# anuragranj/cc

Measured on NVIDIA H100. Metric: train-step triplets/sec at 256x832x6lvl, higher is better.
Workload: dtype f32

## Files before the change

cc_b200/csrc/conv_tc.cu:

```cuda
#include "conv.cuh"

#ifndef CCB_CPU_SIM

#include <cuda.h>
#include <cudaTypedefs.h>

namespace ccb {

constexpr int TC_M = 128;
constexpr int TC_NMAX = 128;
constexpr int TC_KC = 8;
constexpr int TC_MAX_STAGES = 4;
constexpr int TC_PRODUCERS = 128;
constexpr int TC_CONSUMER_WARPS = 8;
constexpr int TC_THREADS = TC_PRODUCERS + 32 * TC_CONSUMER_WARPS;
constexpr int TC_MAX_TAPS = 49;
constexpr int TC_PRODUCER_REGS = 72, TC_CONSUMER_REGS = 216;

struct TcArgs {
    CUtensorMap wmap;
    const float* x;
    const float* bias;
    const float* res;
    float* out;
    int B, Cin, Hin, Win;
    int Ntot;
    int Hout, Wout;
    int Hc, Wc;
    int out_stride, out_oy, out_ox;
    int in_stride;
    int ntaps, cpad, Kp;
    int M;
    int act;
    float slope;
    int ktiles, kt_per_split, splits;
    float* partial;
    int tiles_m, tiles_n, units;
    long long out_numel;
    int depth, b_tile_bytes;
    signed char off_y[TC_MAX_TAPS], off_x[TC_MAX_TAPS];
};

__device__ __forceinline__ uint32_t smem_u32(const void* p) { return (uint32_t)__cvta_generic_to_shared(p); }

__device__ __forceinline__ void mbar_init(uint64_t* bar, uint32_t count) {
    asm volatile("mbarrier.init.shared::cta.b64 [%0], %1;" ::"r"(smem_u32(bar)), "r"(count));
}
__device__ __forceinline__ void mbar_arrive(uint64_t* bar) {
    asm volatile("mbarrier.arrive.shared::cta.b64 _, [%0];" ::"r"(smem_u32(bar)) : "memory");
}
__device__ __forceinline__ bool mbar_try(uint64_t* bar, uint32_t parity) {
    uint32_t ok;
    asm volatile(
        "{\n\t"
        ".reg .pred p;\n\t"
        "mbarrier.try_wait.parity.shared::cta.b64 p, [%1], %2;\n\t"
        "selp.u32 %0, 1, 0, p;\n\t"
        "}"
        : "=r"(ok)
        : "r"(smem_u32(bar)), "r"(parity)
        : "memory");
    return ok != 0;
}
__device__ __forceinline__ void mbar_wait(uint64_t* bar, uint32_t parity) {
    uint32_t spins = 0;
    while (!mbar_try(bar, parity)) {
        if (++spins > (1u << 26)) asm volatile("trap;");
    }
}
__device__ __forceinline__ void fence_proxy_async() { asm volatile("fence.proxy.async.shared::cta;" ::: "memory"); }
__device__ __forceinline__ void fence_barrier_init() { asm volatile("fence.mbarrier_init.release.cluster;" ::: "memory"); }
__device__ __forceinline__ void mbar_arrive_expect_tx(uint64_t* bar, uint32_t bytes) {
    asm volatile("mbarrier.arrive.expect_tx.shared::cta.b64 _, [%0], %1;" ::"r"(smem_u32(bar)), "r"(bytes) : "memory");
}
__device__ __forceinline__ void tma_load_3d(void* dst, const CUtensorMap* map, uint64_t* bar, int c0, int c1, int c2) {
    asm volatile(
        "cp.async.bulk.tensor.3d.shared::cluster.global.mbarrier::complete_tx::bytes [%0], [%1, {%3, %4, %5}], [%2];"
        ::"r"(smem_u32(dst)), "l"(map), "r"(smem_u32(bar)), "r"(c0), "r"(c1), "r"(c2)
        : "memory");
}
__device__ __forceinline__ void tma_prefetch_map(const CUtensorMap* map) {
    asm volatile("prefetch.tensormap [%0];" ::"l"(map) : "memory");
}
__device__ __forceinline__ void cp_async_4(uint32_t dst, const float* src, bool valid) {
    asm volatile("cp.async.ca.shared.global [%0], [%1], 4, %2;" ::"r"(dst), "l"(src), "r"(valid ? 4 : 0) : "memory");
}
__device__ __forceinline__ void cp_async_arrive(uint64_t* bar) {
    asm volatile("cp.async.mbarrier.arrive.noinc.shared::cta.b64 [%0];" ::"r"(smem_u32(bar)) : "memory");
}
__device__ __forceinline__ void cp_async_wait_all() { asm volatile("cp.async.wait_all;" ::: "memory"); }
__device__ __forceinline__ void cp_async_16(uint32_t dst, const void* src, bool valid) {
    asm volatile("cp.async.cg.shared.global [%0], [%1], 16, %2;" ::"r"(dst), "l"(src), "r"(valid ? 16 : 0) : "memory");
}
__device__ __forceinline__ float tf32_hi(float x) {
    uint32_t r;
    asm("cvt.rna.tf32.f32 %0, %1;" : "=r"(r) : "f"(x));
    return __uint_as_float(r);
}

__device__ __forceinline__ uint64_t wg_desc(uint32_t saddr) {
    return (uint64_t)((saddr & 0x3FFFF) >> 4) | ((uint64_t)1 << 16) | ((uint64_t)(1024 >> 4) << 32) | ((uint64_t)1 << 62);
}
__device__ __forceinline__ void wg_fence() { asm volatile("wgmma.fence.sync.aligned;" ::: "memory"); }
__device__ __forceinline__ void wg_commit() { asm volatile("wgmma.commit_group.sync.aligned;" ::: "memory"); }
template <int PENDING>
__device__ __forceinline__ void wg_wait() { asm volatile("wgmma.wait_group.sync.aligned %0;" ::"n"(PENDING) : "memory"); }
template <int R>
__device__ __forceinline__ void wg_fence_regs(float (&d)[R]) {
#pragma unroll
    for (int i = 0; i < R; ++i) asm volatile("" : "+f"(d[i])::"memory");
}
template <int K, int R>
__device__ __forceinline__ void wg_fence_regs(uint32_t (&d)[K][R]) {
#pragma unroll
    for (int k = 0; k < K; ++k)
#pragma unroll
        for (int i = 0; i < R; ++i) asm volatile("" : "+r"(d[k][i])::"memory");
}

__device__ __forceinline__ void wgmma_tf32_rs_n16(float (&d)[8], const uint32_t (&a)[4], uint64_t db) {
    asm volatile(
        "{\n\t.reg .pred p;\n\tsetp.ne.b32 p, 1, 0;\n\t"
        "wgmma.mma_async.sync.aligned.m64n16k8.f32.tf32.tf32 "
        "{%0, %1, %2, %3, %4, %5, %6, %7}, "
        "{%8, %9, %10, %11}, %12, p, 1, 1;\n\t}"
        : "+f"(d[0]), "+f"(d[1]), "+f"(d[2]), "+f"(d[3]), "+f"(d[4]), "+f"(d[5]), "+f"(d[6]), "+f"(d[7])
        : "r"(a[0]), "r"(a[1]), "r"(a[2]), "r"(a[3]), "l"(db));
}
__device__ __forceinline__ void wgmma_tf32_rs_n32(float (&d)[16], const uint32_t (&a)[4], uint64_t db) {
    asm volatile(
        "{\n\t.reg .pred p;\n\tsetp.ne.b32 p, 1, 0;\n\t"
        "wgmma.mma_async.sync.aligned.m64n32k8.f32.tf32.tf32 "
        "{%0, %1, %2, %3, %4, %5, %6, %7, %8, %9, %10, %11, %12, %13, %14, %15}, "
        "{%16, %17, %18, %19}, %20, p, 1, 1;\n\t}"
        : "+f"(d[0]), "+f"(d[1]), "+f"(d[2]), "+f"(d[3]), "+f"(d[4]), "+f"(d[5]), "+f"(d[6]), "+f"(d[7]),
          "+f"(d[8]), "+f"(d[9]), "+f"(d[10]), "+f"(d[11]), "+f"(d[12]), "+f"(d[13]), "+f"(d[14]), "+f"(d[15])
        : "r"(a[0]), "r"(a[1]), "r"(a[2]), "r"(a[3]), "l"(db));
}
__device__ __forceinline__ void wgmma_tf32_rs_n64(float (&d)[32], const uint32_t (&a)[4], uint64_t db) {
    asm volatile(
        "{\n\t.reg .pred p;\n\tsetp.ne.b32 p, 1, 0;\n\t"
        "wgmma.mma_async.sync.aligned.m64n64k8.f32.tf32.tf32 "
        "{%0, %1, %2, %3, %4, %5, %6, %7, %8, %9, %10, %11, %12, %13, %14, %15,"
        " %16, %17, %18, %19, %20, %21, %22, %23, %24, %25, %26, %27, %28, %29, %30, %31}, "
        "{%32, %33, %34, %35}, %36, p, 1, 1;\n\t}"
        : "+f"(d[0]), "+f"(d[1]), "+f"(d[2]), "+f"(d[3]), "+f"(d[4]), "+f"(d[5]), "+f"(d[6]), "+f"(d[7]),
          "+f"(d[8]), "+f"(d[9]), "+f"(d[10]), "+f"(d[11]), "+f"(d[12]), "+f"(d[13]), "+f"(d[14]), "+f"(d[15]),
          "+f"(d[16]), "+f"(d[17]), "+f"(d[18]), "+f"(d[19]), "+f"(d[20]), "+f"(d[21]), "+f"(d[22]), "+f"(d[23]),
          "+f"(d[24]), "+f"(d[25]), "+f"(d[26]), "+f"(d[27]), "+f"(d[28]), "+f"(d[29]), "+f"(d[30]), "+f"(d[31])
        : "r"(a[0]), "r"(a[1]), "r"(a[2]), "r"(a[3]), "l"(db));
}
__device__ __forceinline__ void wgmma_tf32_rs_n128(float (&d)[64], const uint32_t (&a)[4], uint64_t db) {
    asm volatile(
        "{\n\t.reg .pred p;\n\tsetp.ne.b32 p, 1, 0;\n\t"
        "wgmma.mma_async.sync.aligned.m64n128k8.f32.tf32.tf32 "
        "{%0, %1, %2, %3, %4, %5, %6, %7, %8, %9, %10, %11, %12, %13, %14, %15,"
        " %16, %17, %18, %19, %20, %21, %22, %23, %24, %25, %26, %27, %28, %29, %30, %31,"
        " %32, %33, %34, %35, %36, %37, %38, %39, %40, %41, %42, %43, %44, %45, %46, %47,"
        " %48, %49, %50, %51, %52, %53, %54, %55, %56, %57, %58, %59, %60, %61, %62, %63}, "
        "{%64, %65, %66, %67}, %68, p, 1, 1;\n\t}"
        : "+f"(d[0]), "+f"(d[1]), "+f"(d[2]), "+f"(d[3]), "+f"(d[4]), "+f"(d[5]), "+f"(d[6]), "+f"(d[7]),
          "+f"(d[8]), "+f"(d[9]), "+f"(d[10]), "+f"(d[11]), "+f"(d[12]), "+f"(d[13]), "+f"(d[14]), "+f"(d[15]),
          "+f"(d[16]), "+f"(d[17]), "+f"(d[18]), "+f"(d[19]), "+f"(d[20]), "+f"(d[21]), "+f"(d[22]), "+f"(d[23]),
          "+f"(d[24]), "+f"(d[25]), "+f"(d[26]), "+f"(d[27]), "+f"(d[28]), "+f"(d[29]), "+f"(d[30]), "+f"(d[31]),
          "+f"(d[32]), "+f"(d[33]), "+f"(d[34]), "+f"(d[35]), "+f"(d[36]), "+f"(d[37]), "+f"(d[38]), "+f"(d[39]),
          "+f"(d[40]), "+f"(d[41]), "+f"(d[42]), "+f"(d[43]), "+f"(d[44]), "+f"(d[45]), "+f"(d[46]), "+f"(d[47]),
          "+f"(d[48]), "+f"(d[49]), "+f"(d[50]), "+f"(d[51]), "+f"(d[52]), "+f"(d[53]), "+f"(d[54]), "+f"(d[55]),
          "+f"(d[56]), "+f"(d[57]), "+f"(d[58]), "+f"(d[59]), "+f"(d[60]), "+f"(d[61]), "+f"(d[62]), "+f"(d[63])
        : "r"(a[0]), "r"(a[1]), "r"(a[2]), "r"(a[3]), "l"(db));
}
template <int NT>
__device__ __forceinline__ void wgmma_tf32_rs(float (&d)[NT / 2], const uint32_t (&a)[4], uint64_t db) {
    if constexpr (NT == 16) wgmma_tf32_rs_n16(d, a, db);
    else if constexpr (NT == 32) wgmma_tf32_rs_n32(d, a, db);
    else if constexpr (NT == 64) wgmma_tf32_rs_n64(d, a, db);
    else wgmma_tf32_rs_n128(d, a, db);
}

template <int R> __device__ __forceinline__ void wg_regs_dec() { asm volatile("setmaxnreg.dec.sync.aligned.u32 %0;" ::"n"(R)); }
template <int R> __device__ __forceinline__ void wg_regs_inc() { asm volatile("setmaxnreg.inc.sync.aligned.u32 %0;" ::"n"(R)); }

constexpr int TC_TILE_BYTES = TC_KC * TC_M * 16;
constexpr int TC_SMEM_MAX = 227 * 1024;

__device__ __forceinline__ int tile_idx(int row, int chunk) { return row * TC_KC + (chunk ^ (row & 7)); }

__device__ __forceinline__ void tc_split_store(unsigned char* hi, unsigned char* lo, int idx, float4 x) {
    float4 h, l;
    h.x = tf32_hi(x.x); h.y = tf32_hi(x.y); h.z = tf32_hi(x.z); h.w = tf32_hi(x.w);
    ((float4*)hi)[idx] = h;
    l.x = tf32_hi(x.x - h.x); l.y = tf32_hi(x.y - h.y); l.z = tf32_hi(x.z - h.z); l.w = tf32_hi(x.w - h.w);
    ((float4*)lo)[idx] = l;
}

template <typename T> struct TcTiles { T a_hi, a_lo, b_hi, b_lo; };

struct TcRing {
    unsigned char* smem;
    int depth, stage_bytes, b_tile_bytes;
    uint64_t *full, *empty;

    template <typename T>
    __device__ __forceinline__ TcTiles<T> tiles(T base, int s) const {
        const T st = base + s * stage_bytes;
        return {st, st + TC_TILE_BYTES, st + 2 * TC_TILE_BYTES, st + 2 * TC_TILE_BYTES + b_tile_bytes};
    }
    __device__ __forceinline__ TcTiles<unsigned char*> acquire(int it, int s) const {
        if (it >= depth) mbar_wait(&empty[s], ((it / depth) - 1) & 1);
        return tiles(smem, s);
    }
    __device__ __forceinline__ void publish(int s) const { fence_proxy_async(); mbar_arrive(&full[s]); }
};

__device__ __forceinline__ TcRing tc_ring(int depth, int b_tile_bytes, int full_arrivals) {
    CCB_PDL_TRIGGER();
    extern __shared__ __align__(1024) unsigned char smem_raw[];
    unsigned char* smem = smem_raw + ((1024u - (smem_u32(smem_raw) & 1023u)) & 1023u);
    const int stage_bytes = 2 * TC_TILE_BYTES + 2 * b_tile_bytes;
    uint64_t* full = (uint64_t*)(smem + depth * stage_bytes);
    const TcRing r = {smem, depth, stage_bytes, b_tile_bytes, full, full + TC_MAX_STAGES};
    if (threadIdx.x == 0) {
        for (int s = 0; s < depth; ++s) { mbar_init(&r.full[s], full_arrivals); mbar_init(&r.empty[s], TC_CONSUMER_WARPS); }
        fence_barrier_init();
    }
    __syncthreads();
    CCB_PDL_SYNC();
    return r;
}

__device__ __forceinline__ int tc_acc_row(int wg, int wq, int lane, int half) { return wg * 64 + wq * 16 + (lane >> 2) + half * 8; }
__device__ __forceinline__ int tc_acc_col(int lane, int i, int e) { return 8 * i + 2 * (lane & 3) + e; }
__device__ __forceinline__ int tc_acc_reg(int i, int half, int e) { return 4 * i + 2 * half + e; }

struct TcAFrag { uint32_t hi[TC_KC / 2][4], lo[TC_KC / 2][4]; };

__device__ __forceinline__ int tc_a_idx(int r, int k) { return k * TC_M + (r ^ (8 * (k & 3))); }
struct TcAFprop {
    __device__ __forceinline__ static int off(int r0, int t) { return tc_a_idx(r0, t) * 4; }
    __device__ __forceinline__ static int at(int off, int h, int j) { return (off ^ (32 * h)) + 2048 * j; }
};
struct TcAWgrad {
    __device__ __forceinline__ static int idx(int r, int k) { return 32 * r + (k ^ (4 * (r & 7))); }
    __device__ __forceinline__ static int off(int r0, int t) { return idx(r0, t) * 4; }
    __device__ __forceinline__ static int at(int off, int h, int j) { return (off + 1024 * h) ^ (16 * j); }
};
template <typename L>
__device__ __forceinline__ void tc_load_a(const unsigned char* tile, int off, float (&v)[2][8]) {
#pragma unroll
    for (int h = 0; h < 2; ++h)
#pragma unroll
        for (int j = 0; j < 8; ++j) v[h][j] = *(const float*)(tile + L::at(off, h, j));
}
__device__ __forceinline__ void tc_split_a(const float (&v)[2][8], TcAFrag& f) {
#pragma unroll
    for (int ks = 0; ks < TC_KC / 2; ++ks)
#pragma unroll
        for (int i = 0; i < 4; ++i) {
            const float x = v[i & 1][2 * ks + (i >> 1)], h = tf32_hi(x);
            f.hi[ks][i] = __float_as_uint(h);
            f.lo[ks][i] = __float_as_uint(tf32_hi(x - h));
        }
}

__device__ __forceinline__ void tc_consumer_sync() { asm volatile("bar.sync 1, %0;" ::"n"(32 * TC_CONSUMER_WARPS) : "memory"); }

struct TcFpropFeed {
    static constexpr bool split_b = false;
    __device__ __forceinline__ void prep_b(const TcTiles<unsigned char*>&) const {}
};

template <int NT, typename L, typename Feed>
__device__ __forceinline__ void tc_consume_rs(const TcRing& ring, int g, int nkt, int wg, int wq, int lane, const Feed& feed,
                                              float (&acc)[NT / 2]) {
    constexpr bool split_ahead = NT < 128;
#pragma unroll
    for (int j = 0; j < NT / 2; ++j) acc[j] = 0.f;
    const uint32_t base = smem_u32(ring.smem);
    const int a_off = L::off(wg * 64 + wq * 16 + (lane >> 2), lane & 3);
    TcAFrag cur, nxt;
    auto take = [&](int st, uint32_t ph, TcAFrag& f) {
        mbar_wait(&ring.full[st], ph);
        const TcTiles<unsigned char*> t = ring.tiles(ring.smem, st);
        float v[2][8];
        tc_load_a<L>(t.a_hi, a_off, v);
        tc_split_a(v, f);
        if constexpr (Feed::split_b) {
            feed.prep_b(t);
            fence_proxy_async();
            tc_consumer_sync();
        }
    };
    float part[NT / 2];
    int s = g % ring.depth;
    uint32_t phase = (g / ring.depth) & 1;
    if constexpr (split_ahead) {
        if (nkt > 0) take(s, phase, cur);
    }
    for (int it = 0; it < nkt; ++it) {
        if constexpr (!split_ahead) take(s, phase, cur);
        const TcTiles<uint32_t> tl = ring.tiles(base, s);
#pragma unroll
        for (int j = 0; j < NT / 2; ++j) part[j] = 0.f;
        wg_fence();
#pragma unroll
        for (int ks = 0; ks < TC_KC / 2; ++ks) {
            const uint32_t koff = (uint32_t)ks * 32u;
            wgmma_tf32_rs<NT>(part, cur.lo[ks], wg_desc(tl.b_hi + koff));
            wgmma_tf32_rs<NT>(part, cur.hi[ks], wg_desc(tl.b_lo + koff));
        }
#pragma unroll
        for (int ks = 0; ks < TC_KC / 2; ++ks)
            wgmma_tf32_rs<NT>(part, cur.hi[ks], wg_desc(tl.b_hi + (uint32_t)ks * 32u));
        wg_commit();
        const int s1 = s + 1 == ring.depth ? 0 : s + 1;
        const uint32_t phase1 = phase ^ (s1 == 0);
        if constexpr (split_ahead) {
            if (it + 1 < nkt) take(s1, phase1, nxt);
        }
        wg_wait<0>();
        wg_fence_regs(part);
        wg_fence_regs(cur.hi);
        wg_fence_regs(cur.lo);
        if (lane == 0) mbar_arrive(&ring.empty[s]);
#pragma unroll
        for (int j = 0; j < NT / 2; ++j) acc[j] += part[j];
        if constexpr (split_ahead) cur = nxt;
        s = s1;
        phase = phase1;
    }
}

struct TcUnit { int m0, n0, z, kt_beg, nkt; };
template <typename Args>
__device__ __forceinline__ TcUnit tc_unit(const Args& a, int u) {
    TcUnit w;
    w.m0 = (u % a.tiles_m) * TC_M;
    u /= a.tiles_m;
    w.n0 = (u % a.tiles_n) * TC_NMAX;
    w.z = u / a.tiles_n;
    w.kt_beg = w.z * a.kt_per_split;
    w.nkt = max(0, min(a.ktiles, w.kt_beg + a.kt_per_split) - w.kt_beg);
    return w;
}

template <int NT>
__global__ void __launch_bounds__(TC_THREADS, 1) conv_tc_kernel(const __grid_constant__ TcArgs a) {
    const TcRing ring = tc_ring(a.depth, a.b_tile_bytes, TC_PRODUCERS + 1);
    const int tid = threadIdx.x, warp = tid >> 5, lane = tid & 31;
    const long long HWin = (long long)a.Hin * a.Win;

    if (warp < TC_PRODUCERS / 32) {
        wg_regs_dec<TC_PRODUCER_REGS>();
        const int r = tid;
        const int cpt = a.cpad >> 2;
        const int nchunks = a.ntaps * cpt;
        if (r == 0) tma_prefetch_map(&a.wmap);
        int g = 0;
        for (int u = blockIdx.x; u < a.units; u += gridDim.x) {
            const TcUnit w = tc_unit(a, u);
            const int m = w.m0 + r;
            const bool mvalid = m < a.M;
            int b = 0, oy = 0, ox = 0;
            if (mvalid) {
                int hw = a.Hc * a.Wc;
                b = m / hw;
                int rem = m - b * hw;
                oy = rem / a.Wc;
                ox = rem - oy * a.Wc;
            }
            const float* xb = a.x + (long long)b * a.Cin * HWin;
            const int iy0 = oy * a.in_stride, ix0 = ox * a.in_stride;
            for (int it = 0; it < w.nkt; ++it, ++g) {
                const int s = g % ring.depth;
                const int kt = w.kt_beg + it;
                const TcTiles<unsigned char*> t = ring.acquire(g, s);
                if (r == 0) {
                    mbar_arrive_expect_tx(&ring.full[s], 2 * ring.b_tile_bytes);
                    tma_load_3d(t.b_hi, &a.wmap, &ring.full[s], kt * (TC_KC * 4), w.n0, 0);
                    tma_load_3d(t.b_lo, &a.wmap, &ring.full[s], kt * (TC_KC * 4), w.n0, 1);
                }
                const uint32_t at = smem_u32(t.a_hi);
                const int q0 = kt * TC_KC;
                const int tap0 = q0 / cpt, c40 = q0 - tap0 * cpt;
                if (c40 + TC_KC <= cpt) {
                    bool ok = mvalid && tap0 < a.ntaps;
                    int pix = 0;
                    if (ok) {
                        const int iy = iy0 + a.off_y[tap0], ix = ix0 + a.off_x[tap0];
                        ok = (iy >= 0) && (iy < a.Hin) && (ix >= 0) && (ix < a.Win);
                        pix = iy * a.Win + ix;
                    }
                    const float* p = ok ? xb + (long long)(c40 * 4) * HWin + pix : a.x;
                    const int nv = ok ? (a.Cin - c40 * 4) : 0;
#pragma unroll
                    for (int c = 0; c < TC_KC; ++c)
#pragma unroll
                        for (int j = 0; j < 4; ++j) {
                            const bool v = c * 4 + j < nv;
                            cp_async_4(at + 4 * tc_a_idx(r, 4 * c + j), v ? p + (c * 4 + j) * HWin : a.x, v);
                        }
                } else {
                    int q = q0, tap = tap0, c4 = c40;
#pragma unroll
                    for (int c = 0; c < TC_KC; ++c) {
                        const float* p = a.x;
                        int nv = 0;
                        if (mvalid && q < nchunks) {
                            const int iy = iy0 + a.off_y[tap], ix = ix0 + a.off_x[tap];
                            if (iy >= 0 && iy < a.Hin && ix >= 0 && ix < a.Win) {
                                p = xb + (long long)(c4 * 4) * HWin + (iy * a.Win + ix);
                                nv = a.Cin - c4 * 4;
                            }
                        }
#pragma unroll
                        for (int j = 0; j < 4; ++j) {
                            const bool v = j < nv;
                            cp_async_4(at + 4 * tc_a_idx(r, 4 * c + j), v ? p + j * HWin : a.x, v);
                        }
                        ++q;
                        if (++c4 == cpt) { c4 = 0; ++tap; }
                    }
                }
                cp_async_arrive(&ring.full[s]);
            }
        }
        cp_async_wait_all();
    } else {
        wg_regs_inc<TC_CONSUMER_REGS>();
        const int wg = (warp - TC_PRODUCERS / 32) >> 2, wq = warp & 3;
        const long long HWout = (long long)a.Hout * a.Wout;
        int g = 0;
        for (int u = blockIdx.x; u < a.units; u += gridDim.x) {
            const TcUnit w = tc_unit(a, u);
            const int ntile = min(TC_NMAX, a.Ntot - w.n0);
            float acc[NT / 2];
            tc_consume_rs<NT, TcAFprop>(ring, g, w.nkt, wg, wq, lane, TcFpropFeed(), acc);
            g += w.nkt;
#pragma unroll
            for (int half = 0; half < 2; ++half) {
                const int em = w.m0 + tc_acc_row(wg, wq, lane, half);
                if (em >= a.M) continue;
                int hw = a.Hc * a.Wc;
                int eb = em / hw;
                int rem = em - eb * hw;
                int eoy = rem / a.Wc, eox = rem - eoy * a.Wc;
                const long long obase = (long long)eb * a.Ntot * HWout + (long long)(eoy * a.out_stride + a.out_oy) * a.Wout +
                                        (eox * a.out_stride + a.out_ox);
#pragma unroll
                for (int i = 0; i < NT / 8; ++i)
#pragma unroll
                    for (int e = 0; e < 2; ++e) {
                        const int nl = tc_acc_col(lane, i, e);
                        if (nl < ntile) {
                            float o = acc[tc_acc_reg(i, half, e)];
                            const int n = w.n0 + nl;
                            const long long off = obase + (long long)n * HWout;
                            if (a.splits > 1) {
                                a.partial[(long long)w.z * a.out_numel + off] = o;
                            } else {
                                if (a.bias) o += __ldg(a.bias + n);
                                if (a.res) o += __ldg(a.res + off);
                                a.out[off] = apply_act(o, a.act, a.slope);
                            }
                        }
                    }
            }
        }
    }
}

static int roundup(int v, int m) { return (v + m - 1) / m * m; }
static int tc_kp(int ntaps, int Cc) { return ntaps > 0 ? roundup(ntaps * roundup(Cc, 4), TC_KC * 4) : TC_KC * 4; }

static void tc_geometry(int N, int& nt, int& b_tile_bytes, int& depth, int& smem) {
    const int ntile_max = N < TC_NMAX ? N : TC_NMAX;
    nt = 16;
    while (nt < ntile_max) nt <<= 1;
    b_tile_bytes = nt * 128;
    const int stage = 2 * TC_TILE_BYTES + 2 * b_tile_bytes;
    depth = (TC_SMEM_MAX - 2048) / stage;
    if (depth > TC_MAX_STAGES) depth = TC_MAX_STAGES;
    smem = depth * stage + 2048;
}

template <typename Args>
static int tc_launch_kernel(void (*const (&kfns)[4])(const Args), const Args& a, int nt, dim3 grid, int smem, cudaStream_t st,
                            const char* what) {
    auto kfn = kfns[nt == 16 ? 0 : nt == 32 ? 1 : nt == 64 ? 2 : 3];
    cudaFuncSetAttribute(kfn, cudaFuncAttributeMaxDynamicSharedMemorySize, TC_SMEM_MAX);
    CCB_LAUNCH(kfn, grid, dim3(TC_THREADS), smem, st, a);
    return check_launch(what);
}

static void (*const TC_FPROP_KERNELS[4])(const TcArgs) = {conv_tc_kernel<16>, conv_tc_kernel<32>, conv_tc_kernel<64>,
                                                          conv_tc_kernel<128>};

static int tc_weight_map(CUtensorMap* map, const float* wp, int N, int Kp, int nt) {
    static PFN_cuTensorMapEncodeTiled_v12000 encode = [] {
        void* fn = nullptr;
        cudaDriverEntryPointQueryResult q;
        if (cudaGetDriverEntryPointByVersion("cuTensorMapEncodeTiled", &fn, 12000, cudaEnableDefault, &q) != cudaSuccess ||
            q != cudaDriverEntryPointSuccess)
            fn = nullptr;
        return (PFN_cuTensorMapEncodeTiled_v12000)fn;
    }();
    CCB_REQUIRE(encode, CCB_ERR_LAUNCH, "conv_tc: the driver has no cuTensorMapEncodeTiled");
    const cuuint64_t dims[3] = {(cuuint64_t)Kp, (cuuint64_t)N, 2};
    const cuuint64_t strides[2] = {(cuuint64_t)Kp * sizeof(float), (cuuint64_t)N * Kp * sizeof(float)};
    const cuuint32_t box[3] = {TC_KC * 4, (cuuint32_t)nt, 1};
    const cuuint32_t estrides[3] = {1, 1, 1};
    const CUresult rc = encode(map, CU_TENSOR_MAP_DATA_TYPE_FLOAT32, 3, (void*)wp, dims, strides, box, estrides,
                               CU_TENSOR_MAP_INTERLEAVE_NONE, CU_TENSOR_MAP_SWIZZLE_128B, CU_TENSOR_MAP_L2_PROMOTION_L2_256B,
                               CU_TENSOR_MAP_FLOAT_OOB_FILL_NONE);
    CCB_REQUIRE(rc == CUDA_SUCCESS, CCB_ERR_LAUNCH, "conv_tc: cuTensorMapEncodeTiled failed (%d) for N %d Kp %d", (int)rc, N, Kp);
    return CCB_OK;
}

static dim3 tc_persistent_grid(int units) {
    static int sms = [] {
        int dev = 0, n = 0;
        cudaGetDevice(&dev);
        cudaDeviceGetAttribute(&n, cudaDevAttrMultiProcessorCount, dev);
        return n > 0 ? n : NUM_SMS;
    }();
    return dim3(units < sms ? units : sms);
}

static int launch_tc(TcArgs& a, const float* w, int mode, int N, int Cc, int KK, int Ci, const signed char* tap_index,
                     float* wp, float* partial, int splits, cudaStream_t st) {
    a.cpad = roundup(Cc, 4);
    a.Kp = tc_kp(a.ntaps, Cc);
    WPrepDesc p;
    memset(&p, 0, sizeof(p));
    p.w = w; p.wp = wp; p.N = N; p.Cc = Cc; p.KK = KK; p.ntaps = a.ntaps; p.Kp = a.Kp; p.mode = mode; p.Ci = Ci;
    p.layout = WPREP_TC; p.p0 = a.cpad;
    for (int t = 0; t < a.ntaps; ++t) p.tap_index[t] = tap_index[t];
    const float* wpp = nullptr;
    int rc = wprep_get(p, st, &wpp);
    if (rc) return rc;
    a.Ntot = N;
    a.splits = splits;
    a.ktiles = a.Kp / (TC_KC * 4);
    a.kt_per_split = cdiv(a.ktiles, splits);
    a.partial = partial;
    int nt, smem;
    tc_geometry(N, nt, a.b_tile_bytes, a.depth, smem);
    rc = tc_weight_map(&a.wmap, wpp, N, a.Kp, nt);
    if (rc) return rc;
    a.tiles_m = cdiv(a.M, TC_M);
    a.tiles_n = cdiv(N, TC_NMAX);
    a.units = a.tiles_m * a.tiles_n * splits;
    return tc_launch_kernel(TC_FPROP_KERNELS, a, nt, tc_persistent_grid(a.units), smem, st, "conv_tc");
}

struct TcWgradArgs {
    const float* x;
    const float* dy;
    float* out;
    int B, Ci, Hi, Wi, Co, Ho, Wo, kh, kw, stride, pad;
    int cpad, Mtot;
    int P;
    int ktiles, kt_per_split, splits;
    int tiles_m, tiles_n, units;
    int depth, b_tile_bytes;
};

template <int NT>
struct TcWgradFeed {
    static constexpr bool split_b = true;
    int ct;
    __device__ __forceinline__ void prep_b(const TcTiles<unsigned char*>& t) const {
        constexpr int n4 = NT * TC_KC, nthr = 32 * TC_CONSUMER_WARPS;
#pragma unroll
        for (int i = 0; i < (n4 + nthr - 1) / nthr; ++i) {
            const int q = ct + nthr * i;
            if (n4 % nthr == 0 || q < n4) tc_split_store(t.b_hi, t.b_lo, q, ((const float4*)t.a_lo)[q]);
        }
    }
};

template <int NT>
__global__ void __launch_bounds__(TC_THREADS, 1) conv_tc_wgrad_kernel(const TcWgradArgs a) {
    const TcRing ring = tc_ring(a.depth, a.b_tile_bytes, TC_PRODUCERS);
    const int tid = threadIdx.x, warp = tid >> 5, lane = tid & 31;
    const int HWo = a.Ho * a.Wo, HWi = a.Hi * a.Wi;

    if (warp < TC_PRODUCERS / 32) {
        wg_regs_dec<TC_PRODUCER_REGS>();
        const int c = tid & 7, n_lo = tid >> 3, dy_idx = tile_idx(n_lo, c);
        static_assert(1023 + 2 * TC_MAX_STAGES * 8 + TC_PRODUCERS / 32 * 8 * 8 <= 2048, "row-group table past the ring");
        int2* const gtab = (int2*)(ring.empty + TC_MAX_STAGES) + 8 * warp;
        int g = 0;
        for (int u = blockIdx.x; u < a.units; u += gridDim.x) {
            const TcUnit w = tc_unit(a, u);
            const int ntile = min(TC_NMAX, a.Co - w.n0);
            __syncwarp();
            if (lane < 8) {
                const int m = w.m0 + 32 * warp + 4 * lane;
                const int tap = m / a.cpad, ci = m - tap * a.cpad, ky = tap / a.kw, kx = tap - ky * a.kw;
                const int nv = m < a.Mtot ? max(0, min(4, a.Ci - ci)) : 0;
                gtab[lane] = make_int2(ci * HWi + ky * a.Wi + kx, ky | kx << 8 | nv << 16);
            }
            __syncwarp();
            int p = w.kt_beg * (TC_KC * 4) + lane;
            int b = p / HWo, oy = (p - b * HWo) / a.Wo, ox = p - b * HWo - oy * a.Wo;
            const float* dyn = a.dy + (long long)(w.n0 + n_lo) * HWo;
            for (int it = 0; it < w.nkt; ++it, ++g) {
                const int s = g % ring.depth;
                const TcTiles<unsigned char*> t = ring.acquire(g, s);
                const bool pvalid = p < a.P;
                const int iy0 = oy * a.stride - a.pad, ix0 = ox * a.stride - a.pad, pix = iy0 * a.Wi + ix0;
                const float* xb = a.x + (pvalid ? (long long)b * a.Ci * HWi : 0ll);
                asm("" : "+l"(xb));
                uint32_t ab[8];
#pragma unroll
                for (int k = 0; k < 8; ++k) ab[k] = (smem_u32(t.a_hi) + 4096 * warp + 4 * lane) ^ (16 * k);
                int2 gh[4];
#pragma unroll
                for (int q = 0; q < 8; ++q) {
                    if (q % 4 == 0) {
#pragma unroll
                        for (int i = 0; i < 4; ++i) gh[i] = gtab[q + i];
                    }
                    const int2 gq = gh[q % 4];
                    const int ky = gq.y & 0xff, kx = (gq.y >> 8) & 0xff, nv = gq.y >> 16;
                    const bool ok = pvalid && (unsigned)(iy0 + ky) < (unsigned)a.Hi && (unsigned)(ix0 + kx) < (unsigned)a.Wi;
                    const int o = pix + gq.x;
                    if (nv == 4) {
                        const float* src = xb + (ok ? o : 0);
                        const int step = ok ? HWi : 0;
#pragma unroll
                        for (int e = 0; e < 4; ++e)
                            cp_async_4(ab[(4 * q + e) % 8] + 128 * (4 * q + e), src + e * step, ok);
                    } else {
                        const int n = ok ? nv : 0;
#pragma unroll
                        for (int e = 0; e < 4; ++e) {
                            const bool v = e < n;
                            cp_async_4(ab[(4 * q + e) % 8] + 128 * (4 * q + e), xb + (v ? o + e * HWi : 0), v);
                        }
                    }
                }
                const int p0 = p - lane;
                const int bc = __shfl_sync(0xffffffffu, b, 4 * c), remc = __shfl_sync(0xffffffffu, oy * a.Wo + ox, 4 * c);
                const bool cvalid = p0 + 4 * c < a.P;
                const float* dyc = dyn + (long long)bc * a.Co * HWo + remc;
                const uint32_t bt = smem_u32(t.a_lo) + 16 * dy_idx;
#pragma unroll
                for (int j = 0; j < NT / 16; ++j) {
                    const bool v = cvalid && n_lo + 16 * j < ntile;
                    cp_async_16(bt + 2048 * j, v ? dyc + (long long)(16 * j) * HWo : a.dy, v);
                }
                p += TC_KC * 4;
                for (ox += TC_KC * 4; ox >= a.Wo; ox -= a.Wo)
                    if (++oy == a.Ho) { oy = 0; ++b; }
                cp_async_arrive(&ring.full[s]);
            }
        }
        cp_async_wait_all();
    } else {
        wg_regs_inc<TC_CONSUMER_REGS>();
        const int wg = (warp - TC_PRODUCERS / 32) >> 2, wq = warp & 3;
        const int KK = a.kh * a.kw;
        const TcWgradFeed<NT> feed = {tid - TC_PRODUCERS};
        int g = 0;
        for (int u = blockIdx.x; u < a.units; u += gridDim.x) {
            const TcUnit w = tc_unit(a, u);
            const int ntile = min(TC_NMAX, a.Co - w.n0);
            float acc[NT / 2];
            tc_consume_rs<NT, TcAWgrad>(ring, g, w.nkt, wg, wq, lane, feed, acc);
            g += w.nkt;
            float* outp = a.out + (long long)w.z * a.Co * a.Ci * KK;
#pragma unroll
            for (int half = 0; half < 2; ++half) {
                const int em = w.m0 + tc_acc_row(wg, wq, lane, half);
                if (em >= a.Mtot) continue;
                const int etap = em / a.cpad;
                const int eci = em - etap * a.cpad;
                if (eci >= a.Ci) continue;
#pragma unroll
                for (int i = 0; i < NT / 8; ++i)
#pragma unroll
                    for (int e = 0; e < 2; ++e) {
                        const int nl = tc_acc_col(lane, i, e);
                        if (nl < ntile) outp[((long long)(w.n0 + nl) * a.Ci + eci) * KK + etap] = acc[tc_acc_reg(i, half, e)];
                    }
            }
        }
    }
}

static void (*const TC_WGRAD_KERNELS[4])(const TcWgradArgs) = {conv_tc_wgrad_kernel<16>, conv_tc_wgrad_kernel<32>,
                                                                conv_tc_wgrad_kernel<64>, conv_tc_wgrad_kernel<128>};

bool tc_supported(const ccb_conv_desc* d, int op) {
    if (d->kh != d->kw || d->kh * d->kw > TC_MAX_TAPS) return false;
    if (op == CCB_CONV_WGRAD) return (d->Wo % 4 == 0);
    return true;
}
bool tc_profitable(const ccb_conv_desc* d, int op) {
    if (!tc_supported(d, op)) return false;
    const long long M = (op == CCB_CONV_FPROP) ? (long long)d->B * d->Ho * d->Wo : (long long)d->B * d->Hi * d->Wi;
    const long long wsize = (long long)d->Ci * d->Co * d->kh * d->kw;
    return (M >= 128 && wsize >= 64) || (M >= 8 && wsize >= 65536);
}

int tc_plan(const ccb_conv_desc* d, int op, long long& panel_floats) {
    panel_floats = 0;
    if (op == CCB_CONV_WGRAD) {
        const int ktiles = cdiv(d->B * d->Ho * d->Wo, 32);
        const int tiles = cdiv(d->kh * d->kw * roundup(d->Ci, 4), TC_M) * cdiv(d->Co, TC_NMAX);
        int splits = cdiv(2 * NUM_SMS, tiles);
        if (splits > ktiles / 4) splits = ktiles / 4;
        if (splits > 2 * NUM_SMS) splits = 2 * NUM_SMS;
        if (splits < 1) splits = 1;
        return cdiv(ktiles, cdiv(ktiles, splits));
    }
    const bool fp = op == CCB_CONV_FPROP;
    const int s = fp ? 1 : d->stride, N = fp ? d->Co : d->Ci;
    const int Kp = tc_kp(cdiv(d->kh, s) * cdiv(d->kw, s), fp ? d->Ci : d->Co);
    panel_floats = 2ll * N * Kp;
    const long long M = fp ? (long long)d->B * d->Ho * d->Wo : (long long)d->B * cdiv(d->Hi, s) * cdiv(d->Wi, s);
    const long long tiles = (long long)cdiv((int)M, TC_M) * cdiv(N, TC_NMAX);
    const int ktiles = Kp / (TC_KC * 4);
    if (tiles >= NUM_SMS || ktiles < 4) return 1;
    long long splits = (2 * NUM_SMS + tiles - 1) / tiles;
    if (splits > ktiles / 2) splits = ktiles / 2;
    if (splits > 32) splits = 32;
    return splits < 2 ? 1 : (int)splits;
}

int tc_fprop(const ccb_conv_desc* d, const float* x, const float* w, const float* bias, const float* res, float* y,
             float* wp, float* partial, int splits, cudaStream_t st) {
    TcArgs a;
    memset(&a, 0, sizeof(a));
    a.x = x; a.bias = bias; a.res = res; a.out = y;
    a.B = d->B; a.Cin = d->Ci; a.Hin = d->Hi; a.Win = d->Wi;
    a.Hout = d->Ho; a.Wout = d->Wo; a.Hc = d->Ho; a.Wc = d->Wo;
    a.out_stride = 1; a.out_oy = 0; a.out_ox = 0; a.in_stride = d->stride;
    a.ntaps = d->kh * d->kw;
    a.M = d->B * d->Ho * d->Wo;
    a.act = d->act; a.slope = d->slope;
    signed char tix[TC_MAX_TAPS];
    for (int ky = 0; ky < d->kh; ++ky)
        for (int kx = 0; kx < d->kw; ++kx) {
            int t = ky * d->kw + kx;
            a.off_y[t] = (signed char)(ky - d->pad);
            a.off_x[t] = (signed char)(kx - d->pad);
            tix[t] = (signed char)t;
        }
    a.out_numel = (long long)d->B * d->Co * d->Ho * d->Wo;
    int rc = launch_tc(a, w, 0, d->Co, d->Ci, d->kh * d->kw, d->Ci, tix, wp, partial, splits, st);
    if (rc || splits == 1) return rc;
    launch_splitk_reduce(partial, y, bias, res, a.out_numel, splits, d->Ho * d->Wo, d->Co, d->act, d->slope, st);
    return check_launch("conv_tc splitk reduce");
}

int tc_dgrad(const ccb_conv_desc* d, const float* dy, const float* w, const float* bias, const float* res, float* dx,
             float* wp, float* partial, int splits, cudaStream_t st) {
    const int s = d->stride;
    const long long out_numel = (long long)d->B * d->Ci * d->Hi * d->Wi;
    for (int py = 0; py < s && py < d->Hi; ++py)
        for (int px = 0; px < s && px < d->Wi; ++px) {
            const DgradClass k = dgrad_class(d, py, px);
            TcArgs a;
            memset(&a, 0, sizeof(a));
            a.out_numel = out_numel;
            a.x = dy; a.bias = bias; a.res = res; a.out = dx;
            a.B = d->B; a.Cin = d->Co; a.Hin = d->Ho; a.Win = d->Wo;
            a.Hout = d->Hi; a.Wout = d->Wi;
            a.Hc = k.Hc; a.Wc = k.Wc;
            a.out_stride = s; a.out_oy = py; a.out_ox = px; a.in_stride = 1;
            a.M = d->B * a.Hc * a.Wc;
            a.act = d->act; a.slope = d->slope;
            a.ntaps = k.nky * k.nkx;
            signed char tix[TC_MAX_TAPS];
            for (int ty = 0; ty < k.nky; ++ty)
                for (int tx = 0; tx < k.nkx; ++tx) {
                    const int ky = k.ky0 + ty * s, kx = k.kx0 + tx * s, t = ty * k.nkx + tx;
                    a.off_y[t] = (signed char)((py + d->pad - ky) / s);
                    a.off_x[t] = (signed char)((px + d->pad - kx) / s);
                    tix[t] = (signed char)(ky * d->kw + kx);
                }
            int rc = launch_tc(a, w, 1, d->Ci, d->Co, d->kh * d->kw, d->Ci, tix, wp, partial, splits, st);
            if (rc) return rc;
        }
    if (splits > 1) {
        launch_splitk_reduce(partial, dx, bias, res, out_numel, splits, d->Hi * d->Wi, d->Ci, d->act, d->slope, st);
        return check_launch("conv_tc dgrad splitk reduce");
    }
    return CCB_OK;
}

int tc_wgrad(const ccb_conv_desc* d, const float* x, const float* dy, float* dw, float* partial, int splits, cudaStream_t st) {
    TcWgradArgs a;
    memset(&a, 0, sizeof(a));
    a.x = x; a.dy = dy;
    a.B = d->B; a.Ci = d->Ci; a.Hi = d->Hi; a.Wi = d->Wi; a.Co = d->Co; a.Ho = d->Ho; a.Wo = d->Wo;
    a.kh = d->kh; a.kw = d->kw; a.stride = d->stride; a.pad = d->pad;
    a.cpad = roundup(d->Ci, 4);
    a.Mtot = d->kh * d->kw * a.cpad;
    a.P = d->B * d->Ho * d->Wo;
    a.ktiles = cdiv(a.P, 32);
    a.kt_per_split = cdiv(a.ktiles, splits);
    a.splits = splits;
    a.out = splits > 1 ? partial : dw;
    const long long numel = (long long)d->Co * d->Ci * d->kh * d->kw;
    int nt, wsmem;
    tc_geometry(d->Co, nt, a.b_tile_bytes, a.depth, wsmem);
    a.tiles_m = cdiv(a.Mtot, TC_M);
    a.tiles_n = cdiv(d->Co, TC_NMAX);
    a.units = a.tiles_m * a.tiles_n * splits;
    int rc = tc_launch_kernel(TC_WGRAD_KERNELS, a, nt, tc_persistent_grid(a.units), wsmem, st, "conv_tc_wgrad");
    if (rc || a.splits == 1) return rc;
    launch_splitk_reduce(partial, dw, nullptr, nullptr, numel, splits, 1, 1, CCB_ACT_NONE, 0.f, st);
    return check_launch("conv_tc_wgrad_reduce");
}

}

extern "C" int ccb_debug_tc_plan(int N, int* out4) {
    if (N < 1 || !out4) return CCB_ERR_ARG;
    ccb::tc_geometry(N, out4[0], out4[1], out4[2], out4[3]);
    return CCB_OK;
}

#else

namespace ccb {
bool tc_supported(const ccb_conv_desc*, int) { return false; }
bool tc_profitable(const ccb_conv_desc*, int) { return false; }
int tc_plan(const ccb_conv_desc*, int, long long& panel_floats) { panel_floats = 0; return 1; }
int tc_fprop(const ccb_conv_desc*, const float*, const float*, const float*, const float*, float*, float*, float*, int,
             cudaStream_t) { return CCB_ERR_UNSUPPORTED; }
int tc_dgrad(const ccb_conv_desc*, const float*, const float*, const float*, const float*, float*, float*, float*, int,
             cudaStream_t) { return CCB_ERR_UNSUPPORTED; }
int tc_wgrad(const ccb_conv_desc*, const float*, const float*, float*, float*, int, cudaStream_t) { return CCB_ERR_UNSUPPORTED; }
}

extern "C" int ccb_debug_tc_plan(int, int*) { return CCB_ERR_UNSUPPORTED; }

#endif
```

Measured before the change: 64.61.

## Overlap WGMMA stages with double-buffered fragments and order warpgroup issue via named barriers

```diff
diff --git a/cc_b200/csrc/conv_tc.cu b/cc_b200/csrc/conv_tc.cu
--- a/cc_b200/csrc/conv_tc.cu
+++ b/cc_b200/csrc/conv_tc.cu
@@ -4,6 +4,7 @@
 
 #include <cuda.h>
 #include <cudaTypedefs.h>
+#include <type_traits>
 
 namespace ccb {
 
@@ -269,15 +270,38 @@
     __device__ __forceinline__ void prep_b(const TcTiles<unsigned char*>&) const {}
 };
 
+constexpr int TC_BAR_WG0_ISSUED = 2, TC_BAR_WG1_ISSUED = 3;
+template <int ID> __device__ __forceinline__ void tc_token_arrive() {
+    asm volatile("bar.arrive %0, %1;" ::"n"(ID), "n"(32 * TC_CONSUMER_WARPS) : "memory");
+}
+template <int ID> __device__ __forceinline__ void tc_token_wait() {
+    asm volatile("bar.sync %0, %1;" ::"n"(ID), "n"(32 * TC_CONSUMER_WARPS) : "memory");
+}
+
+template <int NT>
+__device__ __forceinline__ void tc_issue_stage(const TcTiles<uint32_t>& tl, const TcAFrag& f, float (&part)[NT / 2]) {
+#pragma unroll
+    for (int j = 0; j < NT / 2; ++j) part[j] = 0.f;
+    wg_fence();
+#pragma unroll
+    for (int ks = 0; ks < TC_KC / 2; ++ks) {
+        const uint32_t koff = (uint32_t)ks * 32u;
+        wgmma_tf32_rs<NT>(part, f.lo[ks], wg_desc(tl.b_hi + koff));
+        wgmma_tf32_rs<NT>(part, f.hi[ks], wg_desc(tl.b_lo + koff));
+    }
+#pragma unroll
+    for (int ks = 0; ks < TC_KC / 2; ++ks)
+        wgmma_tf32_rs<NT>(part, f.hi[ks], wg_desc(tl.b_hi + (uint32_t)ks * 32u));
+    wg_commit();
+}
+
 template <int NT, typename L, typename Feed>
 __device__ __forceinline__ void tc_consume_rs(const TcRing& ring, int g, int nkt, int wg, int wq, int lane, const Feed& feed,
                                               float (&acc)[NT / 2]) {
-    constexpr bool split_ahead = NT < 128;
 #pragma unroll
     for (int j = 0; j < NT / 2; ++j) acc[j] = 0.f;
     const uint32_t base = smem_u32(ring.smem);
     const int a_off = L::off(wg * 64 + wq * 16 + (lane >> 2), lane & 3);
-    TcAFrag cur, nxt;
     auto take = [&](int st, uint32_t ph, TcAFrag& f) {
         mbar_wait(&ring.full[st], ph);
         const TcTiles<unsigned char*> t = ring.tiles(ring.smem, st);
@@ -290,43 +314,70 @@
             tc_consumer_sync();
         }
     };
-    float part[NT / 2];
+    auto retire = [&](int st, float (&part)[NT / 2], TcAFrag& f) {
+        wg_fence_regs(part);
+        wg_fence_regs(f.hi);
+        wg_fence_regs(f.lo);
+        if (lane == 0) mbar_arrive(&ring.empty[st]);
+#pragma unroll
+        for (int j = 0; j < NT / 2; ++j) acc[j] += part[j];
+    };
     int s = g % ring.depth;
     uint32_t phase = (g / ring.depth) & 1;
-    if constexpr (split_ahead) {
-        if (nkt > 0) take(s, phase, cur);
-    }
-    for (int it = 0; it < nkt; ++it) {
-        if constexpr (!split_ahead) take(s, phase, cur);
-        const TcTiles<uint32_t> tl = ring.tiles(base, s);
-#pragma unroll
-        for (int j = 0; j < NT / 2; ++j) part[j] = 0.f;
-        wg_fence();
-#pragma unroll
-        for (int ks = 0; ks < TC_KC / 2; ++ks) {
-            const uint32_t koff = (uint32_t)ks * 32u;
-            wgmma_tf32_rs<NT>(part, cur.lo[ks], wg_desc(tl.b_hi + koff));
-            wgmma_tf32_rs<NT>(part, cur.hi[ks], wg_desc(tl.b_lo + koff));
-        }
-#pragma unroll
-        for (int ks = 0; ks < TC_KC / 2; ++ks)
-            wgmma_tf32_rs<NT>(part, cur.hi[ks], wg_desc(tl.b_hi + (uint32_t)ks * 32u));
-        wg_commit();
-        const int s1 = s + 1 == ring.depth ? 0 : s + 1;
-        const uint32_t phase1 = phase ^ (s1 == 0);
-        if constexpr (split_ahead) {
-            if (it + 1 < nkt) take(s1, phase1, nxt);
-        }
-        wg_wait<0>();
-        wg_fence_regs(part);
-        wg_fence_regs(cur.hi);
-        wg_fence_regs(cur.lo);
-        if (lane == 0) mbar_arrive(&ring.empty[s]);
-#pragma unroll
-        for (int j = 0; j < NT / 2; ++j) acc[j] += part[j];
-        if constexpr (split_ahead) cur = nxt;
-        s = s1;
-        phase = phase1;
+    if constexpr (NT < 128) {
+        TcAFrag f[2];
+        float part[2][NT / 2];
+        int sp = s;
+        auto step = [&](auto B, bool first) {
+            constexpr int b = decltype(B)::value;
+            take(s, phase, f[b]);
+            tc_issue_stage<NT>(ring.tiles(base, s), f[b], part[b]);
+            if (!first) {
+                wg_wait<1>();
+                retire(sp, part[b ^ 1], f[b ^ 1]);
+            }
+            sp = s;
+            s = s + 1 == ring.depth ? 0 : s + 1;
+            phase ^= (s == 0);
+        };
+        auto finish = [&](auto B) {
+            wg_wait<0>();
+            retire(sp, part[decltype(B)::value], f[decltype(B)::value]);
+        };
+        using Set0 = std::integral_constant<int, 0>;
+        using Set1 = std::integral_constant<int, 1>;
+        if (nkt > 0) {
+            step(Set0(), true);
+            for (int it = 1;; it += 2) {
+                if (it == nkt) { finish(Set0()); break; }
+                step(Set1(), false);
+                if (it + 1 == nkt) { finish(Set1()); break; }
+                step(Set0(), false);
+            }
+        }
+    } else {
+        constexpr bool ordered = !Feed::split_b;
+        TcAFrag f;
+        float part[NT / 2];
+        for (int it = 0; it < nkt; ++it) {
+            take(s, phase, f);
+            if constexpr (ordered) {
+                if (wg == 1) tc_token_wait<TC_BAR_WG0_ISSUED>();
+                else if (it > 0) tc_token_wait<TC_BAR_WG1_ISSUED>();
+            }
+            tc_issue_stage<NT>(ring.tiles(base, s), f, part);
+            if constexpr (ordered) {
+                if (wg == 0) tc_token_arrive<TC_BAR_WG0_ISSUED>();
+                else tc_token_arrive<TC_BAR_WG1_ISSUED>();
+            }
+            wg_wait<0>();
+            retire(s, part, f);
+            s = s + 1 == ring.depth ? 0 : s + 1;
+            phase ^= (s == 0);
+        }
+        if constexpr (ordered) {
+            if (wg == 0 && nkt > 0) tc_token_wait<TC_BAR_WG1_ISSUED>();
+        }
     }
 }
 
@@ -353,7 +404,7 @@
         wg_regs_dec<TC_PRODUCER_REGS>();
         const int r = tid;
         const int cpt = a.cpad >> 2;
-        const int nchunks = a.ntaps * cpt;
+        const int hwin = a.Hin * a.Win;
         if (r == 0) tma_prefetch_map(&a.wmap);
         int g = 0;
         for (int u = blockIdx.x; u < a.units; u += gridDim.x) {
@@ -382,44 +433,48 @@
                 const uint32_t at = smem_u32(t.a_hi);
                 const int q0 = kt * TC_KC;
                 const int tap0 = q0 / cpt, c40 = q0 - tap0 * cpt;
+                auto tap_src = [&](int tap, int c4, const float*& p, int& step) {
+                    const bool real = tap < a.ntaps;
+                    const int t = real ? tap : 0;
+                    const int iy = iy0 + a.off_y[t], ix = ix0 + a.off_x[t];
+                    const bool ok = mvalid && real && (unsigned)iy < (unsigned)a.Hin && (unsigned)ix < (unsigned)a.Win;
+                    p = xb + (ok ? c4 * 4 * hwin + iy * a.Win + ix : 0);
+                    step = ok ? hwin : 0;
+                };
                 if (c40 + TC_KC <= cpt) {
-                    bool ok = mvalid && tap0 < a.ntaps;
-                    int pix = 0;
-                    if (ok) {
-                        const int iy = iy0 + a.off_y[tap0], ix = ix0 + a.off_x[tap0];
-                        ok = (iy >= 0) && (iy < a.Hin) && (ix >= 0) && (ix < a.Win);
-                        pix = iy * a.Win + ix;
+                    const float* p;
+                    int step;
+                    tap_src(tap0, c40, p, step);
+                    const int nv = a.Cin - c40 * 4;
+                    if (nv >= TC_KC * 4) {
+#pragma unroll
+                        for (int k = 0; k < TC_KC * 4; ++k) cp_async_4(at + 4 * tc_a_idx(r, k), p + k * step, step != 0);
+                    } else {
+#pragma unroll
+                        for (int k = 0; k < TC_KC * 4; ++k)
+                            cp_async_4(at + 4 * tc_a_idx(r, k), p + min(k, nv - 1) * step, step != 0 && k < nv);
                     }
-                    const float* p = ok ? xb + (long long)(c40 * 4) * HWin + pix : a.x;
-                    const int nv = ok ? (a.Cin - c40 * 4) : 0;
-#pragma unroll
-                    for (int c = 0; c < TC_KC; ++c)
-#pragma unroll
-                        for (int j = 0; j < 4; ++j) {
-                            const bool v = c * 4 + j < nv;
-                            cp_async_4(at + 4 * tc_a_idx(r, 4 * c + j), v ? p + (c * 4 + j) * HWin : a.x, v);
+                } else {
+                    auto chunks = [&](auto whole4) {
+                        int tap = tap0, c4 = c40;
+#pragma unroll
+                        for (int c = 0; c < TC_KC; ++c) {
+                            const float* p;
+                            int step;
+                            tap_src(tap, c4, p, step);
+                            const int nv = a.Cin - c4 * 4;
+#pragma unroll
+                            for (int j = 0; j < 4; ++j) {
+                                if constexpr (decltype(whole4)::value)
+                                    cp_async_4(at + 4 * tc_a_idx(r, 4 * c + j), p + j * step, step != 0);
+                                else
+                                    cp_async_4(at + 4 * tc_a_idx(r, 4 * c + j), p + min(j, nv - 1) * step, step != 0 && j < nv);
+                            }
+                            if (++c4 == cpt) { c4 = 0; ++tap; }
                         }
-                } else {
-                    int q = q0, tap = tap0, c4 = c40;
-#pragma unroll
-                    for (int c = 0; c < TC_KC; ++c) {
-                        const float* p = a.x;
-                        int nv = 0;
-                        if (mvalid && q < nchunks) {
-                            const int iy = iy0 + a.off_y[tap], ix = ix0 + a.off_x[tap];
-                            if (iy >= 0 && iy < a.Hin && ix >= 0 && ix < a.Win) {
-                                p = xb + (long long)(c4 * 4) * HWin + (iy * a.Win + ix);
-                                nv = a.Cin - c4 * 4;
-                            }
-                        }
-#pragma unroll
-                        for (int j = 0; j < 4; ++j) {
-                            const bool v = j < nv;
-                            cp_async_4(at + 4 * tc_a_idx(r, 4 * c + j), v ? p + j * HWin : a.x, v);
-                        }
-                        ++q;
-                        if (++c4 == cpt) { c4 = 0; ++tap; }
-                    }
+                    };
+                    if ((a.Cin & 3) == 0) chunks(std::true_type());
+                    else chunks(std::false_type());
                 }
                 cp_async_arrive(&ring.full[s]);
             }
```

Result: faster. 70.15, median of 6 (+8.6%).
